# zondie17/LoRAStencil

Hardware: AMD Instinct MI355X
Metric: GStencils/s (higher is better)
Workload: dtype f64; 1 GPU; star2d1r 16384x16384 fp64, 2697 sweeps (lorastencil_2d star2d1r 16384 16384 2697); parallelism=single GPU, kernel=stencil2d_wg_kernel, variant=direct, normalised_taps=True, graph_replay=False

## Files before the change

### include/lorastencil.h

```cpp
#ifndef LORASTENCIL_H
#define LORASTENCIL_H

#include <stddef.h>
#include <stdint.h>

#ifdef __cplusplus
extern "C" {
#endif

#define LORA_VERSION 100

#define LORA_OK 0
#define LORA_EINVAL (-1)
#define LORA_EUNSUPPORTED (-2)
#define LORA_EHIP (-3)
#define LORA_ENOMEM (-4)
#define LORA_ENODEVICE (-5)

typedef enum lora_shape {
    LORA_1D1R = 0,
    LORA_1D2R = 1,
    LORA_STAR2D1R = 2,
    LORA_BOX2D1R = 3,
    LORA_STAR2D3R = 4,
// ... 89 lines not shown
int lora_last_run_info(lora_run_info *info);

typedef struct lora_plan lora_plan;

int lora_plan_create(lora_plan **plan, int shape, int dtype, const int *dims, const double *params);
int lora_plan_set_weights(lora_plan *plan, const double *weights, int count);
int lora_plan_get_weights(const lora_plan *plan, double *weights, int count);
int lora_plan_set_variant(lora_plan *plan, int variant);
int lora_plan_set_boundary(lora_plan *plan, int boundary);
int lora_set_default_boundary(int boundary);
int lora_plan_set_source(lora_plan *plan, const void *d_source);
const double *lora_set_default_source(const double *padded_host_source);
int lora_set_default_normalize(int on);
int lora_set_default_leap3(int on);
int lora_set_default_coarse1(int on);
int lora_set_default_mgfuse(int on);
int lora_plan_set_option(lora_plan *plan, const char *key, int value);
int lora_plan_get_option(const lora_plan *plan, const char *key, int *value);
size_t lora_plan_padded_bytes(const lora_plan *plan);
const char *lora_plan_kernel_name(const lora_plan *plan);
const char *lora_plan_kernel_signature(const lora_plan *plan);

int lora_plan_step(lora_plan *plan, const void *d_in, void *d_out, void *stream);
int lora_plan_step_region(lora_plan *plan, const void *d_in, void *d_out, int begin, int end, void *stream);
int lora_plan_region_granularity(const lora_plan *plan);
int lora_plan_step2(lora_plan *plan, const void *d_in, void *d_out, void *stream);
int lora_plan_step2_region(lora_plan *plan, const void *d_in, void *d_out, int begin, int end, void *stream);
int lora_plan_stepk(lora_plan *plan, const void *d_in, void *d_out, void *stream);
int lora_plan_stepk_region(lora_plan *plan, const void *d_in, void *d_out, int begin, int end, void *stream);
int lora_plan_stepn_region(lora_plan *plan, int napps, const void *d_in, void *d_out, int begin, int end, void *stream);
int lora_plan_stepn_region2(lora_plan *plan, int napps, const void *d_in, void *d_out, int begin0, int end0, int begin1, int end1,
                            void *stream);
int lora_debug_span_cover(int tiles_x, int tiles_y, int depth, int S, int slots, int team, int *cover, int *workgroups, int *max_steps);
enum lora_cut_kind {
    LORA_CUT_FIXED = 1,
    LORA_CUT_MODEL,
    LORA_CUT_RANGES2,
    LORA_CUT_SLOW,
    LORA_CUT_DEALT,
    LORA_CUT_SPANS,
    LORA_CUT_TEAMS,
    LORA_CUT_TEAMS_FINER
};
int lora_debug_cut_cover(int kernel, int K, int tiles_x, int tiles_y, int h, int begin, int end, int begin2, int end2, int slots,
                         int fused_z_chunk, int spans3, int *cover, int *workgroups, int *max_steps, int *kind);
enum lora_halo_mode { LORA_HALO_COPY = 0, LORA_HALO_ZERO = 1, LORA_HALO_WRAP = 2 };
int lora_plan_halo(lora_plan *plan, void *d_dst, const void *d_src, int mode, void *stream);
int lora_copy_block_f64(void *d_dst, long dst_ld, const void *d_src, long src_ld, long rows, long cols, void *stream);
int lora_plan_run(lora_plan *plan, void *d_buf0, void *d_buf1, int times, void *stream);
int lora_plan_prepare_run(lora_plan *plan, int times);
typedef struct lora_run_profile {
    int fused_launches;
    int apps_per_fused_launch;
    int two_launches;
    int single_launches;
    float fused_ms;
    float two_ms;
    float single_ms;
} lora_run_profile;
int lora_plan_run_profiled(lora_plan *plan, void *d_buf0, void *d_buf1, int times, void *stream,
                           lora_run_profile *profile);

int lora_plan_leapfrog_depth(const lora_plan *plan);
int lora_plan_step_leapfrog(lora_plan *plan, const void *d_cur, void *d_prev, double c, void *stream);
int lora_plan_step_leapfrog_region(lora_plan *plan, const void *d_cur, void *d_prev, double c, int begin, int end, void *stream);
int lora_plan_step2_leapfrog(lora_plan *plan, const void *d_prev, const void *d_cur, void *d_out1, void *d_out2, double c,
// ... 246 lines not shown
```

### lorastencil_amd/_lib.py

```python
from __future__ import annotations

import ctypes
import os

_HERE = os.path.dirname(os.path.abspath(__file__))
LIB_PATH = os.path.join(_HERE, "lib", "liblorastencil_hip.so")

LORA_OK = 0
LORA_EINVAL = -1
LORA_EUNSUPPORTED = -2
LORA_EHIP = -3
LORA_ENOMEM = -4
LORA_ENODEVICE = -5

F64 = 0
BF16 = 1
VARIANT_AUTO, VARIANT_DIRECT, VARIANT_MFMA = 0, 1, 2
BC_REFERENCE, BC_DIRICHLET, BC_PERIODIC = 0, 1, 2

_dp = ctypes.POINTER(ctypes.c_double)
_ip = ctypes.POINTER(ctypes.c_int)
_vp = ctypes.c_void_p


# ... 180 lines not shown
    "lora_block_create": (ctypes.c_int, [ctypes.POINTER(_vp), ctypes.POINTER(BlockDesc), ctypes.POINTER(SlabComm)]),
    "lora_block_destroy": (None, [_vp]),
    "lora_block_info": (ctypes.c_int, [_vp, ctypes.POINTER(BlockInfo)]),
    "lora_block_load": (ctypes.c_int, [_vp, _vp]),
    "lora_block_run": (ctypes.c_int, [_vp, ctypes.c_int]),
    "lora_block_run_many": (ctypes.c_int, [ctypes.POINTER(_vp), ctypes.c_int, ctypes.c_int]),
    "lora_block_sync": (ctypes.c_int, [_vp]),
    "lora_block_store": (ctypes.c_int, [_vp, _vp]),
    "lora_block_buffer": (_vp, [_vp, ctypes.c_int]),
    "lora_block_stream": (_vp, [_vp]),
    "lora_block_comm_stream": (_vp, [_vp]),
    "lora_block_plan": (_vp, [_vp]),
    "lora_run_host_blocks": (ctypes.c_int, [ctypes.c_int, ctypes.c_int, _vp, _vp, _dp, ctypes.c_int, ctypes.POINTER(ctypes.c_int),
                                            ctypes.POINTER(ctypes.c_int), ctypes.c_int, _vp]),
    "lora_run_host_multi": (ctypes.c_int, [ctypes.c_int, ctypes.c_int, _vp, _vp, _dp, ctypes.c_int, _ip, ctypes.c_int,
                                           ctypes.c_int, ctypes.POINTER(RunInfo)]),
    "lora_plan_run_profiled": (ctypes.c_int, [_vp, _vp, _vp, ctypes.c_int, _vp, ctypes.POINTER(RunProfile)]),
    "lora_plan_padded_bytes": (ctypes.c_size_t, [_vp]),
    "lora_plan_kernel_name": (ctypes.c_char_p, [_vp]),
    "lora_plan_step": (ctypes.c_int, [_vp, _vp, _vp, _vp]),
    "lora_plan_step_region": (ctypes.c_int, [_vp, _vp, _vp, ctypes.c_int, ctypes.c_int, _vp]),
    "lora_plan_region_granularity": (ctypes.c_int, [_vp]),
    "lora_plan_step2": (ctypes.c_int, [_vp, _vp, _vp, _vp]),
    "lora_plan_halo": (ctypes.c_int, [_vp, _vp, _vp, ctypes.c_int, _vp]),
    "lora_copy_block_f64": (ctypes.c_int, [_vp, ctypes.c_long, _vp, ctypes.c_long, ctypes.c_long, ctypes.c_long, _vp]),
    "lora_plan_stepk": (ctypes.c_int, [_vp, _vp, _vp, _vp]),
    "lora_plan_step2_region": (ctypes.c_int, [_vp, _vp, _vp, ctypes.c_int, ctypes.c_int, _vp]),
    "lora_plan_stepk_region": (ctypes.c_int, [_vp, _vp, _vp, ctypes.c_int, ctypes.c_int, _vp]),
    "lora_plan_stepn_region": (ctypes.c_int, [_vp, ctypes.c_int, _vp, _vp, ctypes.c_int, ctypes.c_int, _vp]),
    "lora_plan_prepare_run": (ctypes.c_int, [_vp, ctypes.c_int]),
    "lora_plan_stepn_region2": (ctypes.c_int, [_vp, ctypes.c_int, _vp, _vp, ctypes.c_int, ctypes.c_int, ctypes.c_int, ctypes.c_int, _vp]),
    "lora_debug_span_cover": (ctypes.c_int, [ctypes.c_int] * 6 + [ctypes.POINTER(ctypes.c_int), ctypes.POINTER(ctypes.c_int), ctypes.POINTER(ctypes.c_int)]),
    "lora_debug_cut_cover": (ctypes.c_int, [ctypes.c_int] * 12 + [ctypes.POINTER(ctypes.c_int)] * 4),
    "lora_plan_run": (ctypes.c_int, [_vp, _vp, _vp, ctypes.c_int, _vp]),
    "lora_plan_stats": (ctypes.c_int, [_vp, _vp, ctypes.c_int, ctypes.c_int, ctypes.POINTER(GridStats), _vp]),
    "lora_plan_diff": (ctypes.c_int, [_vp, _vp, _vp, ctypes.c_int, ctypes.c_int, ctypes.POINTER(GridDiff), _vp]),
    "lora_plan_residual": (ctypes.c_int, [_vp, _vp, ctypes.c_int, ctypes.c_int, ctypes.POINTER(GridDiff), _vp]),
    "lora_plan_residual_src": (ctypes.c_int, [_vp, _vp, _vp, ctypes.c_int, ctypes.c_int, ctypes.POINTER(GridDiff), _vp]),
    "lora_debug_residual_cover": (ctypes.c_int, [_vp, ctypes.c_int, ctypes.c_int, ctypes.POINTER(ctypes.c_int), ctypes.POINTER(ctypes.c_int)]),
    "lora_grid_stats_merge": (None, [ctypes.POINTER(GridStats), ctypes.POINTER(GridStats)]),
    "lora_plan_run_until": (ctypes.c_int, [_vp, _vp, _vp, ctypes.POINTER(Until), ctypes.POINTER(UntilResult), _vp]),
    "lora_run_host_until": (ctypes.c_int, [ctypes.c_int, ctypes.c_int, _vp, _vp, _dp, _ip, ctypes.POINTER(Until),
                                           ctypes.POINTER(UntilResult), ctypes.c_int, ctypes.POINTER(RunInfo)]),
    "lora_plan_leapfrog_depth": (ctypes.c_int, [_vp]),
    "lora_plan_step_leapfrog": (ctypes.c_int, [_vp, _vp, _vp, ctypes.c_double, _vp]),
    "lora_plan_step_leapfrog_region": (ctypes.c_int, [_vp, _vp, _vp, ctypes.c_double, ctypes.c_int, ctypes.c_int, _vp]),
    "lora_plan_step2_leapfrog": (ctypes.c_int, [_vp, _vp, _vp, _vp, _vp, ctypes.c_double, _vp]),
    "lora_plan_step2_leapfrog_region": (ctypes.c_int, [_vp, _vp, _vp, _vp, _vp, ctypes.c_double, ctypes.c_int, ctypes.c_int, _vp]),
    "lora_plan_run_leapfrog": (ctypes.c_int, [_vp, _vp, _vp, ctypes.c_double, ctypes.c_int, _vp]),
    "lora_plan_prepare_leapfrog": (ctypes.c_int, [_vp, ctypes.c_int]),
    "lora_plan_step_leapfrog_src": (ctypes.c_int, [_vp, _vp, _vp, _vp, ctypes.c_double, ctypes.c_double, _vp]),
    "lora_plan_step_leapfrog_src_region": (ctypes.c_int, [_vp, _vp, _vp, _vp, ctypes.c_double, ctypes.c_double, ctypes.c_int, ctypes.c_int,
                                                          _vp]),
    "lora_plan_step2_leapfrog_src": (ctypes.c_int, [_vp, _vp, _vp, _vp, _vp, _vp, ctypes.c_double, ctypes.c_double, ctypes.c_double,
                                                    ctypes.c_double, _vp]),
    "lora_plan_step2_leapfrog_src_region": (ctypes.c_int, [_vp, _vp, _vp, _vp, _vp, _vp, ctypes.c_double, ctypes.c_double, ctypes.c_double,
                                                           ctypes.c_double, ctypes.c_int, ctypes.c_int, _vp]),
    "lora_plan_run_leapfrog_src": (ctypes.c_int, [_vp, _vp, _vp, _vp, _dp, _dp, ctypes.c_int, ctypes.c_int, _vp]),
    "lora_chebyshev_coeffs": (ctypes.c_int, [ctypes.c_double, ctypes.c_int, ctypes.c_int, _dp, _dp]),
    "lora_plan_wave_depth": (ctypes.c_int, [_vp]),
    "lora_plan_step_wave": (ctypes.c_int, [_vp, _vp, _vp, _vp, ctypes.c_double, ctypes.c_double, _vp]),
    "lora_plan_step_wave_region": (ctypes.c_int, [_vp, _vp, _vp, _vp, ctypes.c_double, ctypes.c_double, ctypes.c_int, ctypes.c_int, _vp]),
    "lora_plan_step2_wave": (ctypes.c_int, [_vp, _vp, _vp, _vp, _vp, _vp, ctypes.c_double, ctypes.c_double, _vp]),
    "lora_plan_step2_wave_region": (ctypes.c_int, [_vp, _vp, _vp, _vp, _vp, _vp, ctypes.c_double, ctypes.c_double, ctypes.c_int, ctypes.c_int,
                                                   _vp]),
    "lora_plan_run_wave": (ctypes.c_int, [_vp, _vp, _vp, _vp, ctypes.c_double, ctypes.c_double, ctypes.c_int, _vp]),
# ... 90 lines not shown
```

### lorastencil_amd/csrc/capi.cpp

```cpp
#include <hip/hip_runtime.h>

#include <cstring>
#include <string>
#include <vector>

#include "engine.h"
#include "spans.h"

namespace lora {

static thread_local std::string g_last_error;
static thread_local lora_run_info g_last_info = {};

void set_last_error(const char *what, hipError_t e) {
    g_last_error = std::string(what) + ": " + hipGetErrorName(e) + " (" + hipGetErrorString(e) + ")";
}

void set_last_error_text(const char *text) { g_last_error = text ? text : ""; }
void set_last_run_info(const lora_run_info &info) { g_last_info = info; }

#define LORA_HIP_TRY(expr)                      \
    do {                                        \
        hipError_t e__ = (expr);                \
        if (e__ != hipSuccess) {                \
// ... 300 lines not shown
        d.pop_back();
    }
    return sc;
}

static Schedule plan_schedule(lora_plan *plan, int times, bool allocate) {
    const int K = run_depth(plan->p, times);
    Schedule sc = run_schedule(plan->p, times, K, true);
    if (sc.scratch && !(allocate ? ensure_scratch(plan) : plan->scratch.ready(lora_plan_padded_bytes(plan))))
        sc = run_schedule(plan->p, times, K, false);
    return sc;
}

struct RunMarks {
    hipEvent_t ev[4] = {nullptr, nullptr, nullptr, nullptr};
    int fused_launches = 0, two_launches = 0, single_launches = 0;
};

int lora_debug_span_cover(int tiles_x, int tiles_y, int depth, int S, int slots, int team, int *cover, int *workgroups, int *max_steps) {
    if (tiles_x < 1 || tiles_y < 1 || depth < 1 || S < 1 || slots < 1 || !cover) return LORA_EINVAL;
    if (team && tiles_x > slots) return LORA_EUNSUPPORTED;
    constexpr unsigned kTeams2 = lora::bf16_lanes_rules(4).decodes;
    lora::Cut3 c{};
    c.z_end = depth;
    c.tiles_x = tiles_x;
    c.tiles_y = tiles_y;
    const long wgs = team ? lora::cut3_set_teams(c, depth, S, slots, team == 2 ? kTeams2 : 0u) : lora::cut3_set_spans(c, depth, S, slots);
    if (wgs <= 0) return LORA_EUNSUPPORTED;
    if (workgroups) *workgroups = (int) wgs;
    const bool ok = team == 2 ? lora::cut3_walk<kTeams2>(c, S, wgs, depth, cover, max_steps) : lora::cut3_walk<0u>(c, S, wgs, depth, cover, max_steps);
    return ok ? LORA_OK : LORA_EHIP;
}

int lora_debug_cut_cover(int kernel, int K, int tiles_x, int tiles_y, int h, int begin, int end, int begin2, int end2, int slots,
                         int fused_z_chunk, int spans3, int *cover, int *workgroups, int *max_steps, int *kind) {
    static_assert(LORA_CUT_FIXED == lora::CUT3_KIND_FIXED && LORA_CUT_TEAMS_FINER == lora::CUT3_KIND_TEAMS_FINER, "one list of layouts");
    if ((kernel != 0 && kernel != 1) || (K != 2 && K != 4) || tiles_x < 1 || tiles_y < 1 || slots < 1 || !cover) return LORA_EINVAL;
    if (begin < 0 || end > h || end < begin || (end2 > begin2 && (begin2 < 0 || end2 > h)) || (end == begin && end2 <= begin2)) return LORA_EINVAL;
    const lora::CutRules R = kernel ? lora::bf16_lanes_rules(K) : lora::lanes3_rules(K);
    const long plane = ((long) tiles_y * ((kernel ? 64 : 32) - 2 * K) + 4) * (120L * tiles_x + 8);
    lora::Cut3 c;
    const long wgs = lora::cut3_plan(R, tiles_x, tiles_y, plane, begin, end, begin2, end2, slots, fused_z_chunk, spans3, c, kind);
    if (wgs <= 0) return LORA_EUNSUPPORTED;
    if (workgroups) *workgroups = (int) wgs;
    const bool ok = kernel ? lora::cut3_walk<lora::bf16_lanes_rules(4).decodes>(c, R.S, wgs, h, cover, max_steps)
                           : lora::cut3_walk<lora::lanes3_rules(4).decodes>(c, R.S, wgs, h, cover, max_steps);
    return ok ? LORA_OK : LORA_EHIP;
}

int lora_plan_stepn_region2(lora_plan *plan, int napps, const void *d_in, void *d_out, int begin0, int end0, int begin1, int end1,
                            void *stream) {
    if (!plan || napps < 1) return LORA_EINVAL;
    const bool apart = end0 <= begin1 || end1 <= begin0;
    if (plan->p.lanes3_active && (napps == 4 || napps == 2) && end0 > begin0 && end1 > begin1 && apart)
        return lora::launch_apps(plan->p, {napps, begin0, end0, begin1, end1}, d_in, d_out, static_cast<hipStream_t>(stream));
    if (end0 > begin0)
        if (int rc = lora_plan_stepn_region(plan, napps, d_in, d_out, begin0, end0, stream)) return rc;
    return end1 > begin1 ? lora_plan_stepn_region(plan, napps, d_in, d_out, begin1, end1, stream) : LORA_OK;
}

static int torus_radius(int nd) { return nd == 1 ? 4 : (nd == 2 ? 3 : 1); }
static const int *torus_pads(int nd) {
    static const int h1[1] = {4}, h2[2] = {4, 4}, h3[3] = {1, 2, 4};
    return nd == 1 ? h1 : (nd == 2 ? h2 : h3);
}

// ... 398 lines not shown
```

### lorastencil_amd/csrc/engine.h

```cpp
#pragma once

#include <hip/hip_runtime_api.h>

#include <string>

#include "lorastencil.h"

namespace lora {

int shape_ndim(int shape);
int shape_ntaps(int shape);
int default_params(int shape, double *params);
int effective_weights(int shape, const double *params, double *weights);
int factorize_7x7(const double *params, double u[4][7], double v[4][7], double *residual_max);
int svd_7x7(const double *W, double u[7][7], double v[7][7], double sigma[7]);
int separable_27(const float *w27, float *cba9);
int separable_27d(const double *w27, double *cba9);
int mfma_factors_27(const float *cba9, float *scale, float *cba9_normalised);

enum TapSet2D { TAPS2D_DIAMOND = 0, TAPS2D_STAR = 1, TAPS2D_BOX = 2 };
enum TapSet3D { TAPS3D_STAR = 0, TAPS3D_BOX = 1, TAPS3D_SEP = 2 };

struct Taps9 {
    double w[9];
// ... 89 lines not shown
inline bool has_fused_kernels(const Plan &p, bool odd_ok) {
    return p.ndim == 1 || ((p.ndim == 3 || p.variant == LORA_VARIANT_DIRECT) && (!p.generic || odd_ok));
}
inline bool has_fused_kernels(const Plan &p) {
    return has_fused_kernels(p, p.ndim == 2 ? p.stream2 && p.boundary == LORA_BC_REFERENCE : p.lanes3_active != 0);
}
inline bool mfma3_applies(const Plan &p) {
    return p.dtype == LORA_BF16 && p.mfma3_valid && p.boundary == LORA_BC_REFERENCE && p.steps_per_launch_req != 1;
}

void plan_refresh(Plan &p);

hipError_t launch_1d(const Plan &p, const double *in, double *out, int begin, int end, hipStream_t s);
hipError_t launch_1d_fused(const Plan &p, int K, const double *in, double *out, int begin, int end, hipStream_t s);
const char *kernel_name_1d_fused(const Plan &p);
hipError_t launch_2d_direct(const Plan &p, const double *in, double *out, int begin, int end, hipStream_t s);
hipError_t launch_2d_mfma(const Plan &p, const double *in, double *out, int begin, int end, hipStream_t s);
hipError_t launch_2d_fused2(const Plan &p, const double *in, double *out, int begin, int end, hipStream_t s);
enum HaloMode { HALO_COPY = 0, HALO_ZERO = 1, HALO_WRAP = 2 };
hipError_t launch_halo(const Plan &p, void *dst, const void *src, int mode, hipStream_t s);
hipError_t launch_copy_block(double *dst, long dst_ld, const double *src, long src_ld, long rows, long cols, hipStream_t s);
hipError_t launch_ring_wrap(int dtype, int nd, const int *dims, const int *ring, void *ptr, hipStream_t s);
hipError_t launch_copy_interior(int dtype, int nd, const int *dims, void *dst, const int *pad_dst, const void *src, const int *pad_src,
                                hipStream_t s);
const char *kernel_name_2d_fused2(const Plan &p);
hipError_t launch_2d_stream(const Plan &p, int K, const double *in, double *out, int begin, int end, hipStream_t s);
const char *kernel_name_2d_stream(const Plan &p);
int stream_rows_per_chunk(const Plan &p, int K, int rows_total, int strips);
int stream_strip_width(int K);
hipError_t launch_2d_wg(const Plan &p, int K, const double *in, double *out, int begin, int end, hipStream_t s);
const char *kernel_name_2d_wg(const Plan &p);
void prepare_2d_wg(const Plan &p);
int wg_strip_width(int K);
hipError_t launch_3d(const Plan &p, const double *in, double *out, int begin, int end, hipStream_t s);
hipError_t launch_3d_fused2(const Plan &p, const double *in, double *out, int begin, int end, hipStream_t s);
const char *kernel_name_3d_fused2(const Plan &p);
hipError_t launch_3d_stream(const Plan &p, int K, const double *in, double *out, const double *halo_src, int parity,
                            int begin, int end, hipStream_t s);
const char *kernel_name_3d_stream(const Plan &p);
hipError_t launch_3d_lanes(const Plan &p, int K, const double *in, double *out, int begin, int end, hipStream_t s, int begin2 = 0, int end2 = 0);
const char *kernel_name_3d_lanes(const Plan &p);
bool prepare_3d_lanes(const Plan &p);
int stream3_waves(const Plan &p, int K, int pipe);
hipError_t launch_2d_generic(const Plan &p, const double *in, double *out, int begin, int end, hipStream_t s);
hipError_t launch_3d_generic(const Plan &p, const double *in, double *out, int begin, int end, hipStream_t s);
const char *kernel_name_generic(const Plan &p);
hipError_t launch_3d_bf16(const Plan &p, const void *in, void *out, int begin, int end, hipStream_t s);
const char *kernel_name_3d_bf16(const Plan &p);
hipError_t launch_3d_bf16_fused2(const Plan &p, const void *in, void *out, int begin, int end, hipStream_t s);
const char *kernel_name_3d_bf16_fused2(const Plan &p);
hipError_t launch_3d_bf16_lanes(const Plan &p, int K, const void *in, void *out, int begin, int end, hipStream_t s, int begin2 = 0, int end2 = 0);
const char *kernel_name_3d_bf16_lanes(const Plan &p);
bool prepare_3d_bf16_lanes(const Plan &p);
hipError_t launch_3d_bf16_mfma2(const Plan &p, const void *in, void *out, int begin, int end, hipStream_t s);
const char *kernel_name_3d_bf16_mfma2(const Plan &p);

enum ReduceKind { KIND_F64X2 = 0, KIND_F64X1 = 1, KIND_BF16X8 = 2, KIND_CELL = 3 };
constexpr int kReduceMaxGroups = 1024;
struct ReduceRecord {
    double f[4];
    long long i[2];
};
struct ReduceArgs {
    long total, chunk;
    int ppr, e1;
    int q0, col_lo, col_hi;
// ... 260 lines not shown
```

### lorastencil_amd/csrc/kernels_2d_wg.hip

```cpp
#include <hip/hip_runtime.h>

#include <algorithm>

#include "device_common.h"
#include "rows_2d.h"

namespace lora {

struct ArgsWG {
    const double *in;
    double *out;
    int ld, m, n;
    int row_begin, row_end;
    int strips;
    int outw;
    int rim;
    int rows_i, groups_i, chunks_i;
    int rows_e, groups_e, chunks_e;
    int prio_split;
    int prio_shift;
#ifdef LORA_DIAGNOSTICS
    long long *stamps;
#endif
};

namespace {

constexpr int kRowW = 512;
constexpr int kBufW = 520;

typedef unsigned int u32x4 __attribute__((ext_vector_type(4)));

__host__ __device__ constexpr int wg_halo_levels(int K, bool DIRI) { return DIRI ? K - 1 : K / 2 - 1; }
__host__ __device__ constexpr int wg_lds_doubles(int K, int D, bool DIRI) { return (D + 1) * kRowW + (K - 1) * 2 * kBufW + wg_halo_levels(K, DIRI) * 2 * kRowW + 8; }

template <int EVAL, int KL, int S, int D, int WPS, bool DIRI>
__global__ __launch_bounds__(256 * S, WPS) void stencil2d_wg_kernel(const ArgsWG a, const Taps49 W, const LowRankTaps F) {
    constexpr int K = KL * S, NS = D + 1;
    static_assert(NS == 4 || NS == 2, "ring slots: a power of two");
    static_assert(K % 2 == 0, "fused launches move an even number of levels");
    __shared__ __attribute__((aligned(128))) double lds[wg_lds_doubles(K, D, DIRI)];
    double *const ring = lds;
    double *const rb = lds + NS * kRowW;

    const int lane = threadIdx.x & 63;
    const int wv = __builtin_amdgcn_readfirstlane(threadIdx.x >> 6);
    const int stage = S == 1 ? 0 : (wv >> 2);
    const int wq = wv & 3;
    const int t = wq * 64 + lane;
    const bool first = stage == 0;

    const int blk = xcd_contiguous(blockIdx.x, gridDim.x);
    int strip, chunk, rows, groups;
    if (blk < a.rim * a.chunks_e) {
        const int q = blk / a.chunks_e;
        chunk = blk - q * a.chunks_e;
        strip = a.rim == 2 ? (q == 0 ? 0 : a.strips - 1) : q;
        rows = a.rows_e;
        groups = a.groups_e;
    } else {
        const int b2 = blk - a.rim * a.chunks_e, ni = a.strips - a.rim;
        chunk = b2 / ni;
        strip = 1 + (b2 - chunk * ni);
        rows = a.rows_i;
        groups = a.groups_i;
    }
#ifdef LORA_DIAGNOSTICS
    if (a.stamps && threadIdx.x == 0) {
        a.stamps[4 * blockIdx.x + 0] = __builtin_amdgcn_s_memrealtime();
        a.stamps[4 * blockIdx.x + 2] = __builtin_amdgcn_s_getreg(63492) | ((long long) __builtin_amdgcn_s_getreg(63508) << 32);
        a.stamps[4 * blockIdx.x + 3] = ((long long) strip << 32) | (unsigned) chunk;
    }
#endif
    const int i0 = a.row_begin + chunk * rows;
    const int j0 = strip * a.outw;
    const int row_hi = min(i0 + rows, a.row_end);
    groups = min(groups, (row_hi - i0 + 7 * K - 1 + 6) / 7);
    const bool col_edge = j0 - 3 * K < 0 || j0 + kRowW > a.n;

    const int gcol = min(max(j0 - 3 * K + 4 + 2 * t, 0), a.n + 6);
    auto issue = [&](int r) {
        const int pr = min(max(i0 - 3 * K + 4 + r, 0), a.m + 7);
        __builtin_amdgcn_global_load_lds((const __attribute__((address_space(1))) void *) (a.in + (size_t) pr * a.ld + gcol),
                                         (__attribute__((address_space(3))) void *) (ring + (r & (NS - 1)) * kRowW + wq * 128), 16, 0, 0);
    };
    const unsigned store_off = t < a.outw / 2 ? 16u * t : 0x80000000u;
    const unsigned row_bytes = (unsigned) (max(min(a.outw, a.n - j0), 0) * 8);
    double *const out_strip = a.out + (j0 + 4);

    for (int k = threadIdx.x; k < (K - 1) * 2 * kBufW / 2 + 4; k += 256 * S) *reinterpret_cast<d2 *>(rb + 2 * k) = (d2){0.0, 0.0};
    if (first)
#pragma unroll
        for (int k = 0; k < D; ++k) issue(k);

    auto run_stage = [&](auto stage_tag) {
        constexpr int STAGE = decltype(stage_tag)::value;
        constexpr bool FIRST = STAGE == 0;
        constexpr int LB = STAGE * KL;
        double pa[KL][7], pb[KL][7];
#pragma unroll
        for (int j = 0; j < KL; ++j)
#pragma unroll
            for (int k = 0; k < 7; ++k) pa[j][k] = pb[j][k] = 0.0;
        const double *const winp = lds + 2 * t;
        constexpr int NC = KL > 1 ? KL - 1 : 1;
        d2 own[NC];
#pragma unroll
        for (int j = 0; j < NC; ++j) own[j] = (d2){0.0, 0.0};
        unsigned cmask0[KL], cmask1[KL];
        constexpr int NH = wg_halo_levels(K, DIRI);
        unsigned hcol[NH > 0 ? NH : 1], hall[NH > 0 ? NH : 1];
        auto edge_state = [&]() {
            int te = t;
            asm volatile("" : "+v"(te));
#pragma unroll
            for (int j = 0; j < KL; ++j) {
                const int c0 = j0 - 3 * K + 3 * (LB + j + 1) + 2 * te;
                cmask0[j] = (unsigned) c0 < (unsigned) a.n ? ~0u : 0u;
                cmask1[j] = (unsigned) (c0 + 1) < (unsigned) a.n ? ~0u : 0u;
                asm volatile("" : "+v"(cmask0[j]), "+v"(cmask1[j]));
            }
            if (FIRST) {
#pragma unroll
                for (int e = 0; e < NH; ++e) {
                    const int c0 = j0 - 3 * K + 3 * (DIRI ? e + 1 : 2 * e + 2) + 2 * te;
                    hall[e] = 8u * (unsigned) min(max(c0 + 4, 0), a.n + 6);
                    hcol[e] = ((unsigned) c0 < (unsigned) a.n && (unsigned) (c0 + 1) < (unsigned) a.n) ? 0x80000000u : hall[e];
                    asm volatile("" : "+v"(hcol[e]), "+v"(hall[e]));
                }
            }
        };
        double *const hb = lds + NS * kRowW + (K - 1) * 2 * kBufW;

        auto step = [&](const int r, auto phase_tag, auto edge_tag) {
            constexpr int P = decltype(phase_tag)::value;
            constexpr bool EDGE = decltype(edge_tag)::value;
            const int par = r & 1;
            if (FIRST) asm volatile("s_waitcnt vmcnt(%0)" ::"n"(EDGE && NH > 0 ? 1 : D - 1) : "memory");
            asm volatile("s_waitcnt lgkmcnt(0)" ::: "memory");
            __builtin_amdgcn_s_barrier();
            asm volatile("" ::: "memory");
            const int cur = par * kBufW, prev = kBufW - cur;
            auto window = [&](const int jj, double (&w)[8]) {
                const int lw = LB + jj + 1;
                const double *const src = lw == 1 ? winp + (r & (NS - 1)) * kRowW : winp + NS * kRowW + (lw - 2) * 2 * kBufW + prev;
                const bool own_pair = jj >= 1;
                if (own_pair) {
                    w[0] = own[jj >= 1 ? jj - 1 : 0].x;
                    w[1] = own[jj >= 1 ? jj - 1 : 0].y;
                }
#pragma unroll
                for (int q = own_pair ? 1 : 0; q < 4; ++q) {
                    const d2 w2 = *reinterpret_cast<const d2 *>(src + 2 * q);
                    w[2 * q] = w2.x;
                    w[2 * q + 1] = w2.y;
                }
            };
            constexpr bool kEarly = !EDGE && EVAL == EVAL_NEST;
            double win[8];
#pragma unroll
            for (int j = KL - 1; j >= 0; --j) {
                const int l = LB + j + 1;
                const int row = i0 - 3 * K - 4 * l + 1 + r;
                const bool to_global = l == K;
                if (!kEarly || j == KL - 1) window(j, win);
                d2 h = {0.0, 0.0};
                if (EDGE && !to_global && ((l & 1) == 0 || DIRI))
                    h = *reinterpret_cast<const d2 *>(winp + NS * kRowW + (K - 1) * 2 * kBufW + ((DIRI ? l - 1 : l / 2 - 1) * 2 + par) * kRowW);
                pa[j][(P + 6) % 7] = 0.0;
                pb[j][(P + 6) % 7] = 0.0;
                if constexpr (kEarly) {
                    double t0[4], t1[4];
                    nest_profiles(win, t0, t1, F);
                    __builtin_amdgcn_sched_barrier(0);
                    if (j > 0) window(j - 1, win);
                    __builtin_amdgcn_sched_barrier(0);
                    nest_scatter<7, P>(6, t0, t1, pa[j], pb[j], F);
                    if (j > 0) {
                        if (j - 1 == 0) asm volatile("" ::"v"(win[0]), "v"(win[1]));
                        asm volatile("" ::"v"(win[2]), "v"(win[3]), "v"(win[4]), "v"(win[5]), "v"(win[6]), "v"(win[7]));
                    }
                } else {
                    apply_row<EVAL, 7, P>(6, win, pa[j], pb[j], W, F);
                }
                d2 v;
                v.x = pa[j][P];
                v.y = pb[j][P];
                if (to_global) {
                    const bool live = row >= i0 && row < row_hi;
                    const __amdgpu_buffer_rsrc_t dst = __builtin_amdgcn_make_buffer_rsrc(
                        out_strip + (size_t) (max(row, 0) + 4) * a.ld, 0, live ? row_bytes : 0u, 0x00020000);
                    __builtin_amdgcn_raw_buffer_store_b128(__builtin_bit_cast(u32x4, v), dst, store_off, 0, kStoreNT);
                } else {
                    if (EDGE) {
                        const unsigned rmask = (unsigned) row < (unsigned) a.m ? ~0u : 0u;
                        const unsigned m0 = cmask0[j] & rmask, m1 = cmask1[j] & rmask;
                        const u32x4 vb = __builtin_bit_cast(u32x4, v), hb4 = __builtin_bit_cast(u32x4, h);
                        u32x4 o;
                        o.x = (vb.x & m0) | (hb4.x & ~m0);
                        o.y = (vb.y & m0) | (hb4.y & ~m0);
                        o.z = (vb.z & m1) | (hb4.z & ~m1);
                        o.w = (vb.w & m1) | (hb4.w & ~m1);
                        v = __builtin_bit_cast(d2, o);
                    }
                    *reinterpret_cast<d2 *>(const_cast<double *>(winp) + NS * kRowW + (l - 1) * 2 * kBufW + cur) = v;
                    if (j < KL - 1) own[j < KL - 1 ? j : 0] = v;
                }
                __builtin_amdgcn_sched_barrier(0);
            }
            asm volatile("" ::: "memory");
            if (FIRST) {
                if (EDGE) {
#pragma unroll
                    for (int e = 0; e < NH; ++e) {
                        const int row1 = i0 - 3 * K - 4 * (DIRI ? e + 1 : 2 * e + 2) + 1 + (r + 1);
                        const int pr = min(max(row1 + 4, 0), a.m + 7);
                        const __amdgpu_buffer_rsrc_t hsrc = __builtin_amdgcn_make_buffer_rsrc(
                            const_cast<double *>(a.in) + (size_t) pr * a.ld, 0, (unsigned) a.ld * 8u, 0x00020000);
#if defined(__HIP_DEVICE_COMPILE__)
                        __builtin_amdgcn_raw_ptr_buffer_load_lds(
                            hsrc, (__attribute__((address_space(3))) void *) (hb + (e * 2 + (par ^ 1)) * kRowW + wq * 128), 16,
                            (unsigned) row1 < (unsigned) a.m ? hcol[e] : hall[e], 0, 0, 0);
#else
                        (void) hsrc;
                        (void) hb;
#endif
                    }
                }
                issue(r + D);
            }
            __builtin_amdgcn_sched_barrier(0);
        };
        auto group = [&](const int r0, auto edge_tag) {
            step(r0 + 0, std::integral_constant<int, 0>{}, edge_tag);
            step(r0 + 1, std::integral_constant<int, 1>{}, edge_tag);
            step(r0 + 2, std::integral_constant<int, 2>{}, edge_tag);
            step(r0 + 3, std::integral_constant<int, 3>{}, edge_tag);
            step(r0 + 4, std::integral_constant<int, 4>{}, edge_tag);
            step(r0 + 5, std::integral_constant<int, 5>{}, edge_tag);
            step(r0 + 6, std::integral_constant<int, 6>{}, edge_tag);
        };

        const int lo0 = i0 - 3 * K - 4 * (K - 1) + 1, hi0 = i0 - 3 * K - 4 + 1 + 6;
        int g1 = lo0 >= 0 ? 0 : (-lo0 + 6) / 7, g2 = hi0 >= a.m ? 0 : (a.m - hi0 + 6) / 7 - 1;
        if (col_edge) g1 = groups;
        g1 = min(g1, groups);
        g2 = min(max(g2, g1), groups);
        const int cls = a.prio_split > 0 ? ((int) blockIdx.x >= a.prio_split ? 1 : 0) : -1;
        auto slice = [&]() {
            if (cls >= 0) {
                const int bit = (int) (__builtin_amdgcn_s_memrealtime() >> a.prio_shift) & 1;
                if (bit != cls)
                    __builtin_amdgcn_s_setprio(1);
                else
                    __builtin_amdgcn_s_setprio(0);
            }
        };
        int g = 0;
        if constexpr (STAGE > 0) {
            const int idle = min(STAGE * KL, groups);
            for (int q = 0; q < 7 * idle; ++q) {
                asm volatile("s_waitcnt lgkmcnt(0)" ::: "memory");
                __builtin_amdgcn_s_barrier();
            }
            g = idle;
        }
        edge_state();
        for (; g < g1; ++g) {
            slice();
            group(7 * g, std::true_type{});
        }
        for (; g < g2; ++g) {
            slice();
            group(7 * g, std::false_type{});
        }
        if constexpr (KL > 1) edge_state();
        for (; g < groups; ++g) {
            slice();
            group(7 * g, std::true_type{});
        }
    };
    static_assert(S >= 1 && S <= 4, "stages");
    if (stage == 0) run_stage(std::integral_constant<int, 0>{});
    if constexpr (S >= 2)
        if (stage == 1) run_stage(std::integral_constant<int, 1>{});
    if constexpr (S >= 3)
        if (stage == 2) run_stage(std::integral_constant<int, 2>{});
    if constexpr (S >= 4)
        if (stage == 3) run_stage(std::integral_constant<int, 3>{});
#ifdef LORA_DIAGNOSTICS
    if (a.stamps && threadIdx.x == 0) a.stamps[4 * blockIdx.x + 1] = __builtin_amdgcn_s_memrealtime();
#endif
    asm volatile("s_waitcnt vmcnt(0)" ::: "memory");
}

template <int EVAL, int KL, int S, int D, int WPS, bool DIRI>
int wg_per_cu(int dev) {
    static int per_cu[64] = {0};
    if (dev < 0 || dev >= 64) dev = 0;
    if (per_cu[dev] == 0) {
        int nb = 0;
        if (hipOccupancyMaxActiveBlocksPerMultiprocessor(&nb, stencil2d_wg_kernel<EVAL, KL, S, D, WPS, DIRI>, 256 * S, 0) != hipSuccess || nb < 1) {
            (void) hipGetLastError();
            return 1;
        }
        per_cu[dev] = nb;
    }
    return per_cu[dev];
}

template <int EVAL, int KL, int S, int D, int WPS, bool DIRI>
hipError_t launch_wg_t(const Plan &p, ArgsWG a, int rows_total, hipStream_t s) {
    constexpr int K = KL * S;
    auto kernel = stencil2d_wg_kernel<EVAL, KL, S, D, WPS, DIRI>;
    int dev = 0, cus = 256;
    if (hipGetDevice(&dev) != hipSuccess || dev < 0 || dev >= 64) dev = 0;
    {
        int v = 0;
        if (hipDeviceGetAttribute(&v, hipDeviceAttributeMultiprocessorCount, dev) == hipSuccess && v > 0) cus = v;
    }
    const int per_cu_dev = wg_per_cu<EVAL, KL, S, D, WPS, DIRI>(dev);
    if (rows_total <= 0) return hipSuccess;
    const int lag = 7 * K - 1;
    auto fit = [&](long rows) {
        long g = (rows + lag + 6) / 7;
        if (g < K + 1) g = K + 1;
        return (int) (7 * g - lag);
    };
    a.rim = a.strips >= 3 ? 2 : a.strips;
    const int ni = a.strips - a.rim;
    const int pct = p.wg_edge_pct >= 0 ? p.wg_edge_pct : 60;
    auto rim_rows = [&](int rows_i) { return fit(std::max(1L, (long) (rows_i + lag) * 100 / (100 + pct) - lag)); };
    if (p.wg_rows > 0) {
        a.rows_i = fit(p.wg_rows);
    } else {
        const long slots = (long) per_cu_dev * cus;
        const long min_rows = 3 * lag / 2;
        int best = fit(rows_total);
        for (long c = 1; c <= rows_total; ++c) {
            const int ri = fit((rows_total + c - 1) / c);
            if (ri < min_rows && c > 1) break;
            const int re = ni > 0 ? rim_rows(ri) : ri;
            const long wgs = (long) ni * ((rows_total + ri - 1) / ri) + (long) a.rim * ((rows_total + re - 1) / re);
            if (wgs > slots && c > 1) break;
            best = ri;
        }
        a.rows_i = best;
    }
    a.rows_e = ni > 0 ? rim_rows(a.rows_i) : a.rows_i;
    a.groups_i = (a.rows_i + lag + 6) / 7;
    a.groups_e = (a.rows_e + lag + 6) / 7;
    a.chunks_i = (rows_total + a.rows_i - 1) / a.rows_i;
    a.chunks_e = (rows_total + a.rows_e - 1) / a.rows_e;
    a.prio_split = (p.wg_prio != 0 && per_cu_dev == 2) ? cus : 0;
    a.prio_shift = p.wg_prio > 0 ? p.wg_prio : 12;
    Taps49 w;
    for (int k = 0; k < 49; ++k) w.w[k] = p.w[k];
    LowRankTaps f{};
    for (int tt = 0; tt < 3; ++tt)
        for (int e = 0; e < 7; ++e) {
            f.u[tt][e] = p.lowrank.u[tt][e];
            f.v[tt][e] = p.lowrank.v[tt][e];
        }
    f.rc = p.lowrank_rc;
    if (EVAL == EVAL_NEST)
        for (int k = 0; k < 4; ++k) {
            f.u[0][k] = p.nest_g[k];
            f.v[0][k] = p.nest_a[k];
        }
    const long nblocks = (long) ni * a.chunks_i + (long) a.rim * a.chunks_e;
    if (nblocks > 0x7fffffffL) return hipErrorInvalidValue;
    hipLaunchKernelGGL(kernel, dim3((unsigned) nblocks), dim3(256 * S), 0, s, a, w, f);
    return hipGetLastError();
}

#ifndef LORA_WG_K
#define LORA_WG_K 6
#endif
#ifndef LORA_WG_S
#define LORA_WG_S 2
#endif
template <int EVAL>
hipError_t launch_wg_e(const Plan &p, const ArgsWG &a, int rows_total, hipStream_t s) {
#if LORA_WG_K <= 4
    if (p.boundary == LORA_BC_DIRICHLET) return launch_wg_t<EVAL, LORA_WG_K / 2, 2, 3, 4, true>(p, a, rows_total, s);
#endif
// ... 19 lines not shown
        case EVAL_LR_PYRAMID_SYM_GAP:
            return launch_wg_e<EVAL_LR_PYRAMID_SYM_GAP>(p, a, rows_total, s);
        default:
            break;
    }
    switch (p.tapset) {
        case TAPS2D_DIAMOND:
            return launch_wg_e<TAPS2D_DIAMOND>(p, a, rows_total, s);
        case TAPS2D_STAR:
            return launch_wg_e<TAPS2D_STAR>(p, a, rows_total, s);
        default:
            return launch_wg_e<TAPS2D_BOX>(p, a, rows_total, s);
    }
}

#if LORA_WG_K == 6
hipError_t launch_2d_wg_k4(const Plan &p, ArgsWG a, int rows_total, hipStream_t s);
hipError_t launch_2d_wg_k2(const Plan &p, ArgsWG a, int rows_total, hipStream_t s);

void prepare_2d_wg(const Plan &p) {
    int n = 0;
    if (hipGetDeviceCount(&n) != hipSuccess || n <= 0) {
        (void) hipGetLastError();
        return;
    }
    ArgsWG a{};
    (void) launch_2d_wg_k6(p, a, 0, nullptr);
#ifndef LORA_WG_ONLY_K6
    (void) launch_2d_wg_k4(p, a, 0, nullptr);
    (void) launch_2d_wg_k2(p, a, 0, nullptr);
#endif
}

int wg_strip_width(int K) { return kRowW - 6 * K; }

#ifdef LORA_DIAGNOSTICS
long long *g_wg_stamps = nullptr;
#endif

hipError_t launch_2d_wg(const Plan &p, int K, const double *in, double *out, int begin, int end, hipStream_t s) {
    if (end <= begin) return hipSuccess;
    if (K != 6 && K != 4 && K != 2) return hipErrorInvalidValue;
    if (p.boundary == LORA_BC_PERIODIC || (p.boundary == LORA_BC_DIRICHLET && K == 6)) return hipErrorNotSupported;
    ArgsWG a;
    a.in = in;
    a.out = out;
    a.m = p.dims[0];
    a.n = p.dims[1];
    a.ld = a.n + 8;
    a.row_begin = begin;
    a.row_end = end;
    a.outw = wg_strip_width(K);
    a.strips = (a.n + a.outw - 1) / a.outw;
    a.rim = a.rows_i = a.groups_i = a.chunks_i = a.rows_e = a.groups_e = a.chunks_e = 0;
    a.prio_split = a.prio_shift = 0;
#ifdef LORA_DIAGNOSTICS
    a.stamps = g_wg_stamps;
#endif
#ifdef LORA_WG_ONLY_K6
    return launch_2d_wg_k6(p, a, end - begin, s);
#else
    return K == 6 ? launch_2d_wg_k6(p, a, end - begin, s)
                  : (K == 4 ? launch_2d_wg_k4(p, a, end - begin, s) : launch_2d_wg_k2(p, a, end - begin, s));
#endif
}

const char *kernel_name_2d_wg(const Plan &) { return "stencil2d_wg_kernel"; }
// ... 4 lines not shown
```

Before: 1459 GStencils/s.

## Widen WG strip output by loading tail columns and rebalance rim/interior row layout

```diff
diff --git a/include/lorastencil.h b/include/lorastencil.h
--- a/include/lorastencil.h
+++ b/include/lorastencil.h
@@ -145,6 +145,7 @@
 int lora_plan_stepn_region2(lora_plan *plan, int napps, const void *d_in, void *d_out, int begin0, int end0, int begin1, int end1,
                             void *stream);
 int lora_debug_span_cover(int tiles_x, int tiles_y, int depth, int S, int slots, int team, int *cover, int *workgroups, int *max_steps);
+int lora_debug_wg_layout(lora_plan *plan, int K, int rows, int cus, int per_cu, int *out);
 enum lora_cut_kind {
     LORA_CUT_FIXED = 1,
     LORA_CUT_MODEL,
diff --git a/lorastencil_amd/_lib.py b/lorastencil_amd/_lib.py
--- a/lorastencil_amd/_lib.py
+++ b/lorastencil_amd/_lib.py
@@ -236,6 +236,7 @@
     "lora_plan_stepn_region2": (ctypes.c_int, [_vp, ctypes.c_int, _vp, _vp, ctypes.c_int, ctypes.c_int, ctypes.c_int, ctypes.c_int, _vp]),
     "lora_debug_span_cover": (ctypes.c_int, [ctypes.c_int] * 6 + [ctypes.POINTER(ctypes.c_int), ctypes.POINTER(ctypes.c_int), ctypes.POINTER(ctypes.c_int)]),
     "lora_debug_cut_cover": (ctypes.c_int, [ctypes.c_int] * 12 + [ctypes.POINTER(ctypes.c_int)] * 4),
+    "lora_debug_wg_layout": (ctypes.c_int, [_vp] + [ctypes.c_int] * 4 + [ctypes.POINTER(ctypes.c_int)]),
     "lora_plan_run": (ctypes.c_int, [_vp, _vp, _vp, ctypes.c_int, _vp]),
     "lora_plan_stats": (ctypes.c_int, [_vp, _vp, ctypes.c_int, ctypes.c_int, ctypes.POINTER(GridStats), _vp]),
     "lora_plan_diff": (ctypes.c_int, [_vp, _vp, _vp, ctypes.c_int, ctypes.c_int, ctypes.POINTER(GridDiff), _vp]),
diff --git a/lorastencil_amd/csrc/capi.cpp b/lorastencil_amd/csrc/capi.cpp
--- a/lorastencil_amd/csrc/capi.cpp
+++ b/lorastencil_amd/csrc/capi.cpp
@@ -356,6 +356,12 @@
     return ok ? LORA_OK : LORA_EHIP;
 }
 
+int lora_debug_wg_layout(lora_plan *plan, int K, int rows, int cus, int per_cu, int *out) {
+    if (!plan || !out) return LORA_EINVAL;
+    if (plan->p.ndim != 2) return LORA_EUNSUPPORTED;
+    return lora::wg_layout_debug(plan->p, K, rows, cus, per_cu, out) ? LORA_OK : LORA_EINVAL;
+}
+
 int lora_debug_cut_cover(int kernel, int K, int tiles_x, int tiles_y, int h, int begin, int end, int begin2, int end2, int slots,
                          int fused_z_chunk, int spans3, int *cover, int *workgroups, int *max_steps, int *kind) {
     static_assert(LORA_CUT_FIXED == lora::CUT3_KIND_FIXED && LORA_CUT_TEAMS_FINER == lora::CUT3_KIND_TEAMS_FINER, "one list of layouts");
diff --git a/lorastencil_amd/csrc/engine.h b/lorastencil_amd/csrc/engine.h
--- a/lorastencil_amd/csrc/engine.h
+++ b/lorastencil_amd/csrc/engine.h
@@ -145,6 +145,7 @@
 const char *kernel_name_2d_wg(const Plan &p);
 void prepare_2d_wg(const Plan &p);
 int wg_strip_width(int K);
+bool wg_layout_debug(const Plan &p, int K, int rows, int cus, int per_cu, int out[8]);
 hipError_t launch_3d(const Plan &p, const double *in, double *out, int begin, int end, hipStream_t s);
 hipError_t launch_3d_fused2(const Plan &p, const double *in, double *out, int begin, int end, hipStream_t s);
 const char *kernel_name_3d_fused2(const Plan &p);
diff --git a/lorastencil_amd/csrc/kernels_2d_wg.hip b/lorastencil_amd/csrc/kernels_2d_wg.hip
--- a/lorastencil_amd/csrc/kernels_2d_wg.hip
+++ b/lorastencil_amd/csrc/kernels_2d_wg.hip
@@ -32,7 +32,7 @@
 typedef unsigned int u32x4 __attribute__((ext_vector_type(4)));
 
 __host__ __device__ constexpr int wg_halo_levels(int K, bool DIRI) { return DIRI ? K - 1 : K / 2 - 1; }
-__host__ __device__ constexpr int wg_lds_doubles(int K, int D, bool DIRI) { return (D + 1) * kRowW + (K - 1) * 2 * kBufW + wg_halo_levels(K, DIRI) * 2 * kRowW + 8; }
+__host__ __device__ constexpr int wg_lds_doubles(int K, int D, bool DIRI) { return (D + 1) * kBufW + (K - 1) * 2 * kBufW + wg_halo_levels(K, DIRI) * 2 * kRowW + 8; }
 
 template <int EVAL, int KL, int S, int D, int WPS, bool DIRI>
 __global__ __launch_bounds__(256 * S, WPS) void stencil2d_wg_kernel(const ArgsWG a, const Taps49 W, const LowRankTaps F) {
@@ -41,7 +41,8 @@
     static_assert(K % 2 == 0, "fused launches move an even number of levels");
     __shared__ __attribute__((aligned(128))) double lds[wg_lds_doubles(K, D, DIRI)];
     double *const ring = lds;
-    double *const rb = lds + NS * kRowW;
+    constexpr int RB = NS * kBufW;
+    double *const rb = lds + RB;
 
     const int lane = threadIdx.x & 63;
     const int wv = __builtin_amdgcn_readfirstlane(threadIdx.x >> 6);
@@ -76,13 +77,34 @@
     const int j0 = strip * a.outw;
     const int row_hi = min(i0 + rows, a.row_end);
     groups = min(groups, (row_hi - i0 + 7 * K - 1 + 6) / 7);
-    const bool col_edge = j0 - 3 * K < 0 || j0 + kRowW > a.n;
+    const bool col_edge = j0 - 3 * K + 3 + 128 * wq < 0 || j0 - 3 + 128 * wq + 127 >= a.n;
 
     const int gcol = min(max(j0 - 3 * K + 4 + 2 * t, 0), a.n + 6);
+    const unsigned xoff = 8u * (unsigned) min(max(j0 - 3 * K + 4 + kRowW + 2 * lane, 0), a.n + 6);
+    const unsigned lds_base = (unsigned) (size_t) (__attribute__((address_space(3))) void *) lds;
     auto issue = [&](int r) {
         const int pr = min(max(i0 - 3 * K + 4 + r, 0), a.m + 7);
-        __builtin_amdgcn_global_load_lds((const __attribute__((address_space(1))) void *) (a.in + (size_t) pr * a.ld + gcol),
-                                         (__attribute__((address_space(3))) void *) (ring + (r & (NS - 1)) * kRowW + wq * 128), 16, 0, 0);
+        const double *const grow = a.in + (size_t) pr * a.ld;
+        double *const slot = ring + (r & (NS - 1)) * kBufW;
+#if defined(__HIP_DEVICE_COMPILE__)
+        const unsigned tail = lds_base + 8u * (unsigned) (wq == 3 ? (r & (NS - 1)) * kBufW + kRowW : wg_lds_doubles(K, D, DIRI) - 8);
+        unsigned long long keep_exec;
+        unsigned keep_m0;
+        asm volatile(
+            "s_mov_b64 %0, exec\n\t"
+            "s_mov_b32 %1, m0\n\t"
+            "s_mov_b64 exec, 7\n\t"
+            "s_mov_b32 m0, %4\n\t"
+            "s_nop 0\n\t"
+            "global_load_lds_dwordx4 %2, %3\n\t"
+            "s_mov_b32 m0, %1\n\t"
+            "s_mov_b64 exec, %0"
+            : "=&s"(keep_exec), "=&s"(keep_m0)
+            : "v"(xoff), "s"(grow), "s"(tail)
+            : "memory");
+#endif
+        __builtin_amdgcn_global_load_lds((const __attribute__((address_space(1))) void *) (grow + gcol),
+                                         (__attribute__((address_space(3))) void *) (slot + wq * 128), 16, 0, 0);
     };
     const unsigned store_off = t < a.outw / 2 ? 16u * t : 0x80000000u;
     const unsigned row_bytes = (unsigned) (max(min(a.outw, a.n - j0), 0) * 8);
@@ -130,20 +152,39 @@
                 }
             }
         };
-        double *const hb = lds + NS * kRowW + (K - 1) * 2 * kBufW;
+        double *const hb = lds + RB + (K - 1) * 2 * kBufW;
 
         auto step = [&](const int r, auto phase_tag, auto edge_tag) {
             constexpr int P = decltype(phase_tag)::value;
             constexpr bool EDGE = decltype(edge_tag)::value;
             const int par = r & 1;
-            if (FIRST) asm volatile("s_waitcnt vmcnt(%0)" ::"n"(EDGE && NH > 0 ? 1 : D - 1) : "memory");
+            if (FIRST) asm volatile("s_waitcnt vmcnt(%0)" ::"n"(EDGE && NH > 0 ? 2 : 2 * (D - 1)) : "memory");
             asm volatile("s_waitcnt lgkmcnt(0)" ::: "memory");
             __builtin_amdgcn_s_barrier();
             asm volatile("" ::: "memory");
+            if (FIRST && EDGE) {
+#pragma unroll
+                for (int e = 0; e < NH; ++e) {
+                    const int row1 = i0 - 3 * K - 4 * (DIRI ? e + 1 : 2 * e + 2) + 1 + (r + 1);
+                    const int pr = min(max(row1 + 4, 0), a.m + 7);
+                    const __amdgpu_buffer_rsrc_t hsrc = __builtin_amdgcn_make_buffer_rsrc(
+                        const_cast<double *>(a.in) + (size_t) pr * a.ld, 0, (unsigned) a.ld * 8u, 0x00020000);
+#if defined(__HIP_DEVICE_COMPILE__)
+                    __builtin_amdgcn_raw_ptr_buffer_load_lds(
+                        hsrc, (__attribute__((address_space(3))) void *) (hb + (e * 2 + (par ^ 1)) * kRowW + wq * 128), 16,
+                        (unsigned) row1 < (unsigned) a.m ? hcol[e] : hall[e], 0, 0, 0);
+#else
+                    (void) hsrc;
+                    (void) hb;
+#endif
+                }
+                asm volatile("" ::: "memory");
+                __builtin_amdgcn_sched_barrier(0);
+            }
             const int cur = par * kBufW, prev = kBufW - cur;
             auto window = [&](const int jj, double (&w)[8]) {
                 const int lw = LB + jj + 1;
-                const double *const src = lw == 1 ? winp + (r & (NS - 1)) * kRowW : winp + NS * kRowW + (lw - 2) * 2 * kBufW + prev;
+                const double *const src = lw == 1 ? winp + (r & (NS - 1)) * kBufW : winp + RB + (lw - 2) * 2 * kBufW + prev;
                 const bool own_pair = jj >= 1;
                 if (own_pair) {
                     w[0] = own[jj >= 1 ? jj - 1 : 0].x;
@@ -166,7 +207,7 @@
                 if (!kEarly || j == KL - 1) window(j, win);
                 d2 h = {0.0, 0.0};
                 if (EDGE && !to_global && ((l & 1) == 0 || DIRI))
-                    h = *reinterpret_cast<const d2 *>(winp + NS * kRowW + (K - 1) * 2 * kBufW + ((DIRI ? l - 1 : l / 2 - 1) * 2 + par) * kRowW);
+                    h = *reinterpret_cast<const d2 *>(winp + RB + (K - 1) * 2 * kBufW + ((DIRI ? l - 1 : l / 2 - 1) * 2 + par) * kRowW);
                 pa[j][(P + 6) % 7] = 0.0;
                 pb[j][(P + 6) % 7] = 0.0;
                 if constexpr (kEarly) {
@@ -203,32 +244,13 @@
                         o.w = (vb.w & m1) | (hb4.w & ~m1);
                         v = __builtin_bit_cast(d2, o);
                     }
-                    *reinterpret_cast<d2 *>(const_cast<double *>(winp) + NS * kRowW + (l - 1) * 2 * kBufW + cur) = v;
+                    *reinterpret_cast<d2 *>(const_cast<double *>(winp) + RB + (l - 1) * 2 * kBufW + cur) = v;
                     if (j < KL - 1) own[j < KL - 1 ? j : 0] = v;
                 }
                 __builtin_amdgcn_sched_barrier(0);
             }
             asm volatile("" ::: "memory");
-            if (FIRST) {
-                if (EDGE) {
-#pragma unroll
-                    for (int e = 0; e < NH; ++e) {
-                        const int row1 = i0 - 3 * K - 4 * (DIRI ? e + 1 : 2 * e + 2) + 1 + (r + 1);
-                        const int pr = min(max(row1 + 4, 0), a.m + 7);
-                        const __amdgpu_buffer_rsrc_t hsrc = __builtin_amdgcn_make_buffer_rsrc(
-                            const_cast<double *>(a.in) + (size_t) pr * a.ld, 0, (unsigned) a.ld * 8u, 0x00020000);
-#if defined(__HIP_DEVICE_COMPILE__)
-                        __builtin_amdgcn_raw_ptr_buffer_load_lds(
-                            hsrc, (__attribute__((address_space(3))) void *) (hb + (e * 2 + (par ^ 1)) * kRowW + wq * 128), 16,
-                            (unsigned) row1 < (unsigned) a.m ? hcol[e] : hall[e], 0, 0, 0);
-#else
-                        (void) hsrc;
-                        (void) hb;
-#endif
-                    }
-                }
-                issue(r + D);
-            }
+            if (FIRST) issue(r + D);
             __builtin_amdgcn_sched_barrier(0);
         };
         auto group = [&](const int r0, auto edge_tag) {
@@ -294,6 +316,58 @@
     asm volatile("s_waitcnt vmcnt(0)" ::: "memory");
 }
 
+constexpr int wg_edge_pct_default(int K) { return K >= 6 ? 12 : 60; }
+
+struct WgLayout {
+    int rim, rows_i, chunks_i, rows_e, chunks_e;
+    long workgroups;
+};
+
+inline WgLayout wg_layout(int K, int strips, int rows_total, long slots, int edge_pct, int wg_rows) {
+    const int lag = 7 * K - 1;
+    auto fit = [&](long rows) {
+        long g = (rows + lag + 6) / 7;
+        if (g < K + 1) g = K + 1;
+        return (int) (7 * g - lag);
+    };
+    auto chunks = [&](int rows) { return (rows_total + rows - 1) / rows; };
+    WgLayout L{};
+    L.rim = strips >= 3 ? 2 : strips;
+    const int ni = strips - L.rim;
+    const long ratio = 100 + (edge_pct >= 0 ? edge_pct : wg_edge_pct_default(K));
+    auto rim_target = [&](int ri) { return std::max(1L, (long) (ri + lag) * 100 / ratio - lag); };
+    if (wg_rows > 0) {
+        L.rows_i = fit(wg_rows);
+        L.rows_e = ni > 0 ? fit(rim_target(L.rows_i)) : L.rows_i;
+    } else {
+        const long min_rows = 3 * lag / 2;
+        long best = -1;
+        for (long c = 1; c <= rows_total; ++c) {
+            const int ri = fit((rows_total + c - 1) / c);
+            if (ri < min_rows && c > 1) break;
+            int re = ri;
+            if (ni > 0) {
+                const long ce_max = (slots - (long) ni * chunks(ri)) / L.rim;
+                if (ce_max < 1 && c > 1) break;
+                const long want = (rows_total + rim_target(ri) - 1) / rim_target(ri);
+                const long ce = std::max(1L, std::min(want, ce_max));
+                re = fit((rows_total + ce - 1) / ce);
+            }
+            if ((long) ni * chunks(ri) + (long) L.rim * chunks(re) > slots && c > 1) break;
+            const long score = std::max(100L * (ri + lag), ratio * (re + lag));
+            if (best < 0 || score < best) {
+                best = score;
+                L.rows_i = ri;
+                L.rows_e = re;
+            }
+        }
+    }
+    L.chunks_i = chunks(L.rows_i);
+    L.chunks_e = chunks(L.rows_e);
+    L.workgroups = (long) ni * L.chunks_i + (long) L.rim * L.chunks_e;
+    return L;
+}
+
 template <int EVAL, int KL, int S, int D, int WPS, bool DIRI>
 int wg_per_cu(int dev) {
     static int per_cu[64] = {0};
@@ -321,37 +395,15 @@
     }
     const int per_cu_dev = wg_per_cu<EVAL, KL, S, D, WPS, DIRI>(dev);
     if (rows_total <= 0) return hipSuccess;
-    const int lag = 7 * K - 1;
-    auto fit = [&](long rows) {
-        long g = (rows + lag + 6) / 7;
-        if (g < K + 1) g = K + 1;
-        return (int) (7 * g - lag);
-    };
-    a.rim = a.strips >= 3 ? 2 : a.strips;
+    const WgLayout lay = wg_layout(K, a.strips, rows_total, (long) per_cu_dev * cus, p.wg_edge_pct, p.wg_rows);
+    a.rim = lay.rim;
     const int ni = a.strips - a.rim;
-    const int pct = p.wg_edge_pct >= 0 ? p.wg_edge_pct : 60;
-    auto rim_rows = [&](int rows_i) { return fit(std::max(1L, (long) (rows_i + lag) * 100 / (100 + pct) - lag)); };
-    if (p.wg_rows > 0) {
-        a.rows_i = fit(p.wg_rows);
-    } else {
-        const long slots = (long) per_cu_dev * cus;
-        const long min_rows = 3 * lag / 2;
-        int best = fit(rows_total);
-        for (long c = 1; c <= rows_total; ++c) {
-            const int ri = fit((rows_total + c - 1) / c);
-            if (ri < min_rows && c > 1) break;
-            const int re = ni > 0 ? rim_rows(ri) : ri;
-            const long wgs = (long) ni * ((rows_total + ri - 1) / ri) + (long) a.rim * ((rows_total + re - 1) / re);
-            if (wgs > slots && c > 1) break;
-            best = ri;
-        }
-        a.rows_i = best;
-    }
-    a.rows_e = ni > 0 ? rim_rows(a.rows_i) : a.rows_i;
-    a.groups_i = (a.rows_i + lag + 6) / 7;
-    a.groups_e = (a.rows_e + lag + 6) / 7;
-    a.chunks_i = (rows_total + a.rows_i - 1) / a.rows_i;
-    a.chunks_e = (rows_total + a.rows_e - 1) / a.rows_e;
+    a.rows_i = lay.rows_i;
+    a.rows_e = lay.rows_e;
+    a.groups_i = (a.rows_i + 7 * K - 1 + 6) / 7;
+    a.groups_e = (a.rows_e + 7 * K - 1 + 6) / 7;
+    a.chunks_i = lay.chunks_i;
+    a.chunks_e = lay.chunks_e;
     a.prio_split = (p.wg_prio != 0 && per_cu_dev == 2) ? cus : 0;
     a.prio_shift = p.wg_prio > 0 ? p.wg_prio : 12;
     Taps49 w;
@@ -437,7 +489,17 @@
 #endif
 }
 
-int wg_strip_width(int K) { return kRowW - 6 * K; }
+int wg_strip_width(int K) { return kRowW - 6 * (K - 1); }
+
+bool wg_layout_debug(const Plan &p, int K, int rows, int cus, int per_cu, int out[8]) {
+    if ((K != 6 && K != 4 && K != 2) || rows < 1 || cus < 1 || per_cu < 1 || p.ndim != 2) return false;
+    const int outw = wg_strip_width(K), strips = (p.dims[1] + outw - 1) / outw;
+    const WgLayout L = wg_layout(K, strips, rows, (long) cus * per_cu, p.wg_edge_pct, p.wg_rows);
+    if (L.workgroups > 0x7fffffffL) return false;
+    const int v[8] = {strips, outw, L.rows_i, strips > L.rim ? L.chunks_i : 0, L.rows_e, L.chunks_e, (int) L.workgroups, L.rim};
+    std::copy(v, v + 8, out);
+    return true;
+}
 
 #ifdef LORA_DIAGNOSTICS
 long long *g_wg_stamps = nullptr;
```

After: 1490 GStencils/s (median of 6 runs). 1.02x the previous value.
